# marc345/Dense2Sparse-ViT

Hardware: AMD Instinct MI355X
Metric: training images/s, DeiT-S 224 keep_ratio=0.5 (dense-to-sparse ViT train step, teacher fwd + student fwd/bwd + AdamW) (higher is better)
Workload: dtype f32; 1 GPU; DeiT-Small 224x224 patch16, 1-stage prune keep_ratio=0.5 @ block 3 (196->98 tokens), large LN predictor, kl_div mask loss, per-GPU batch 128; global_batch=128, parallelism=dp1

## Files before the change

dense2sparse-vit_amd/csrc/attention_f32.hip:

```cpp
#include "d2s_common.h"

namespace {

#ifdef D2S_ATTN_STAMPS
__device__ unsigned long long g_attn_stamps[16 * 8192];
#define ASTAMP(i) if (threadIdx.x == 0) { const int L_ = blockIdx.y * gridDim.x + blockIdx.x; if (L_ < 8192) g_attn_stamps[16 * L_ + (i)] = __builtin_amdgcn_s_memtime(); }
#define ASTAMPR(i) if (threadIdx.x == 0) { const int L_ = blockIdx.y * gridDim.x + blockIdx.x; if (L_ < 8192) g_attn_stamps[16 * L_ + (i)] = __builtin_amdgcn_s_memrealtime(); }
#else
#define ASTAMP(i)
#define ASTAMPR(i)
#endif

constexpr int DH = 64;
constexpr int PITCH = 68;

__device__ __forceinline__ void load_rows_regs(const float* __restrict__ base, long ld, int row, int nrows, int half,
                                               float scale, f32x4 (&r)[8]) {
    if (row < nrows) {
        const float* p = base + (long)row * ld + 4 * half;
#pragma unroll
        for (int t = 0; t < 8; ++t) {
            r[t] = *reinterpret_cast<const f32x4*>(p + 8 * t);
#pragma unroll
            for (int j = 0; j < 4; ++j) r[t][j] *= scale;
        }
    } else {
#pragma unroll
        for (int t = 0; t < 8; ++t) r[t] = f32x4{0.f, 0.f, 0.f, 0.f};
    }
}

__device__ __forceinline__ void tile_load(const float* __restrict__ base, long ld, int row0, int nrows, int tid, f32x4 (&r)[2]) {
#pragma unroll
    for (int i = 0; i < 2; ++i) {
        const int f = tid + i * 256, row = row0 + (f >> 4), d4 = (f & 15) * 4;
        r[i] = row < nrows ? *reinterpret_cast<const f32x4*>(base + (long)row * ld + d4) : f32x4{0.f, 0.f, 0.f, 0.f};
    }
}
__device__ __forceinline__ void tile_store(float* __restrict__ S, int tid, const f32x4 (&r)[2]) {
#pragma unroll
    for (int i = 0; i < 2; ++i) {
        const int f = tid + i * 256;
        *reinterpret_cast<f32x4*>(&S[(f >> 4) * PITCH + (f & 15) * 4]) = r[i];
    }
}

__device__ __forceinline__ void mma_lds_reg(const float* __restrict__ S, int l31, int half, const f32x4 (&y)[8], f32x16& acc) {
#pragma unroll
    for (int t = 0; t < 8; ++t) {
        const f32x4 a = *reinterpret_cast<const f32x4*>(&S[l31 * PITCH + 8 * t + 4 * half]);
#pragma unroll
        for (int j = 0; j < 4; ++j) acc = mfma32(a[j], y[t][j], acc);
    }
}
__device__ __forceinline__ void mma_reg_lds(const f32x16& p, const float* __restrict__ S, int l31, int half, f32x16 (&o)[2],
                                            int groups = 4) {
#pragma unroll
    for (int g = 0; g < 4; ++g) {
        if (g < groups) {
#pragma unroll
            for (int r = 4 * g; r < 4 * g + 4; ++r) {
                const float* row = &S[mfma32_row(r, half) * PITCH];
                o[0] = mfma32(p[r], row[l31], o[0]);
                o[1] = mfma32(p[r], row[32 + l31], o[1]);
            }
        }
    }
}

__device__ __forceinline__ void mma_lds_reg_t(const f32x16& p, const float* __restrict__ S, int l31, int half, f32x16 (&o)[2],
                                              int groups = 4) {
#pragma unroll
    for (int g = 0; g < 4; ++g) {
        if (g < groups) {
#pragma unroll
            for (int r = 4 * g; r < 4 * g + 4; ++r) {
                const float* row = &S[mfma32_row(r, half) * PITCH];
                o[0] = mfma32(row[l31], p[r], o[0]);
                o[1] = mfma32(row[32 + l31], p[r], o[1]);
            }
        }
    }
}

struct AttnFwdArgs {
    const float* qkv; float* out; float* lse; float* cls_row;
    const float* policy; float* cinv; const int* cu;
    int n, H; float scale, eps; int total;
};

template <bool POLICY, bool VARLEN>
__global__ __launch_bounds__(256, 3) void attn_fwd_kernel(AttnFwdArgs a) {
    __shared__ __attribute__((aligned(16))) float Ks[32 * PITCH];
    __shared__ __attribute__((aligned(16))) float Vs[32 * PITCH];
    __shared__ float pol_s[32];
    __shared__ __attribute__((aligned(16))) float vred[POLICY ? 16 * 64 : 4];
    __shared__ float vsum_s[64];
    extern __shared__ __attribute__((aligned(16))) float cls_s[];
    const int tid = threadIdx.x, lane = tid & 63, wave = tid >> 6, half = lane >> 5, l31 = lane & 31;
    const int H = a.H;
    ASTAMP(0); ASTAMPR(8);
    int bx, by;
    xcd_remap_2d(bx, by);
    const int b = by / H, h = by % H;
    const long ld = 3L * H * DH;
    const int row_base = VARLEN ? a.cu[b] : 0;
    const int n = VARLEN ? a.cu[b + 1] - row_base : a.n;
    if (VARLEN && bx * 128 >= n) return;
    const long tok0 = VARLEN ? (long)row_base : (long)b * n;
    const float* qb = a.qkv + tok0 * ld + h * DH;
    const float* kb = qb + (long)H * DH;
    const float* vb = kb + (long)H * DH;
    const float* polb = POLICY ? a.policy + (long)b * n : nullptr;
    const float scale = a.scale;
    const int q0 = bx * 128 + wave * 32;
    const bool active = q0 < n;
    const bool want_cls = a.cls_row != nullptr && bx == 0 && wave == 0;
    const int qi = q0 + l31;

    f32x4 qreg[8];
    load_rows_regs(qb, ld, qi, n, half, scale, qreg);

    f32x16 o[2];
#pragma unroll
    for (int r = 0; r < 16; ++r) { o[0][r] = 0.f; o[1][r] = 0.f; }
    float m_run = -INFINITY, l_run = 0.f;
    f32x4 vacc = {0.f, 0.f, 0.f, 0.f};

    const int ntiles = (n + 31) / 32;
    f32x4 kr[2], vr[2];
    float pr = 0.f;
    tile_load(kb, ld, 0, n, tid, kr);
    tile_load(vb, ld, 0, n, tid, vr);
    if (POLICY && tid < 32) pr = tid < n ? polb[tid] : 0.f;
    for (int t = 0; t < ntiles; ++t) {
        __syncthreads();
        tile_store(Ks, tid, kr);
        tile_store(Vs, tid, vr);
        if (POLICY) {
            if (tid < 32) pol_s[tid] = pr;
            vacc += vr[0];
            vacc += vr[1];
        }
        __syncthreads();
        if (t == 0) { ASTAMP(1); }
        if (t == 1) { ASTAMP(2); }
        if (t == 2) { ASTAMP(3); }
        if (t + 1 < ntiles) {
            tile_load(kb, ld, (t + 1) * 32, n, tid, kr);
            tile_load(vb, ld, (t + 1) * 32, n, tid, vr);
            if (POLICY && tid < 32) { const int kj = (t + 1) * 32 + tid; pr = kj < n ? polb[kj] : 0.f; }
        }
        if (!active) continue;
        f32x16 s;
#pragma unroll
        for (int r = 0; r < 16; ++r) s[r] = 0.f;
        mma_lds_reg(Ks, l31, half, qreg, s);
        const int kv0 = t * 32;
        float mt = -INFINITY;
#pragma unroll
        for (int r = 0; r < 16; ++r) {
            if (kv0 + mfma32_row(r, half) >= n) s[r] = -INFINITY;
            mt = fmaxf(mt, s[r]);
        }
        if (want_cls && l31 == 0) {
#pragma unroll
            for (int r = 0; r < 16; ++r) {
                const int key = kv0 + mfma32_row(r, half);
                if (key < n) cls_s[key] = s[r];
            }
        }
        mt = fmaxf(mt, __shfl_xor(mt, 32, 64));
        const float m_new = fmaxf(m_run, mt);
        const float alpha = __expf(m_run - m_new);
        float rs = 0.f;
#pragma unroll
        for (int r = 0; r < 16; ++r) {
            s[r] = __expf(s[r] - m_new);
            if (POLICY) {
                const int kr_ = mfma32_row(r, half);
                s[r] *= (kv0 + kr_ == qi) ? 1.f : pol_s[kr_];
            }
            rs += s[r];
        }
        rs += __shfl_xor(rs, 32, 64);
        l_run = l_run * alpha + rs;
        m_run = m_new;
#pragma unroll
        for (int r = 0; r < 16; ++r) {
            o[0][r] *= alpha;
            o[1][r] *= alpha;
        }
        mma_lds_reg_t(s, Vs, l31, half, o, min(4, (n - kv0 + 7) >> 3));
    }
    ASTAMP(4);
    const float c = POLICY ? a.eps / (float)n : 0.f;
    if (POLICY) {
        *reinterpret_cast<f32x4*>(&vred[(tid >> 4) * 64 + (tid & 15) * 4]) = vacc;
        __syncthreads();
        if (tid < 64) {
            float t = 0.f;
#pragma unroll
            for (int g = 0; g < 16; ++g) t += vred[g * 64 + tid];
            vsum_s[tid] = t * c;
        }
        __syncthreads();
    }
    if (!active) return;
    const float inv_l = 1.0f / (POLICY ? l_run + a.eps : l_run);
    if (qi < n) {
        float* p = a.out + (tok0 + qi) * H * DH + h * DH;
#pragma unroll
        for (int dt = 0; dt < 2; ++dt)
#pragma unroll
            for (int g = 0; g < 4; ++g) {
                f32x4 v;
#pragma unroll
                for (int j = 0; j < 4; ++j) {
                    float num = o[dt][4 * g + j];
                    if (POLICY) num += vsum_s[32 * dt + 8 * g + 4 * half + j];
                    v[j] = num * inv_l;
                }
                *reinterpret_cast<f32x4*>(p + 32 * dt + 8 * g + 4 * half) = v;
            }
    }
    const long stat0 = VARLEN ? (long)h * a.total + row_base : ((long)b * H + h) * n;
    if (half == 0 && qi < n) {
        if (a.lse) a.lse[stat0 + qi] = m_run + logf(POLICY ? l_run + a.eps : l_run);
        if (POLICY && a.cinv) a.cinv[stat0 + qi] = c * inv_l;
    }
    if (want_cls) {
        const float m0 = __shfl(m_run, 0, 64), il0 = __shfl(inv_l, 0, 64);
        float* cr = a.cls_row + stat0;
        for (int j = lane; j < n; j += 64) {
            float e = expf(cls_s[j] - m0);
            if (POLICY) e = e * (j == 0 ? 1.f : polb[j]) + c;
            cr[j] = e * il0;
        }
    }
    ASTAMP(5); ASTAMPR(9);
}

__global__ __launch_bounds__(256) void attn_delta_kernel(const float* __restrict__ out, const float* __restrict__ dout,
                                                         float* __restrict__ delta, long rows, int n, int H) {
    const int lane = threadIdx.x & 63;
    const long row = (long)blockIdx.x * 4 + (threadIdx.x >> 6);
    if (row >= rows) return;
    const long b = row / n, i = row - b * n;
    for (int h = 0; h < H; ++h) {
        const long e = row * H * DH + h * DH + lane;
        const float s = wave_sum(out[e] * dout[e]);
        if (lane == 0) delta[(b * H + h) * n + i] = s;
    }
}

template <bool POLICY>
__global__ __launch_bounds__(256, 3) void attn_bwd_dq_kernel(const float* __restrict__ qkv, const float* __restrict__ dout,
                                                          const float* __restrict__ lse, const float* __restrict__ delta,
                                                          float* __restrict__ dqkv, int n, int H, float scale,
                                                          const float* __restrict__ policy) {
    __shared__ __attribute__((aligned(16))) float Ks[32 * PITCH];
    __shared__ __attribute__((aligned(16))) float Vs[32 * PITCH];
    __shared__ float pol_s[32];
    const int tid = threadIdx.x, lane = tid & 63, wave = tid >> 6, half = lane >> 5, l31 = lane & 31;
    int bx, by;
    xcd_remap_2d(bx, by);
    const int b = by / H, h = by % H;
    const long ld = 3L * H * DH, ldo = (long)H * DH;
    const float* qb = qkv + (long)b * n * ld + h * DH;
    const float* kb = qb + (long)H * DH;
    const float* vb = kb + (long)H * DH;
    const float* dob = dout + (long)b * n * ldo + h * DH;
    const int q0 = bx * 128 + wave * 32;
    const bool active = q0 < n;

    f32x4 qreg[8], doreg[8];
    load_rows_regs(qb, ld, q0 + l31, n, half, scale, qreg);
    load_rows_regs(dob, ldo, q0 + l31, n, half, 1.0f, doreg);
    const bool qok = q0 + l31 < n;
    const float lse_i = qok ? lse[((long)b * H + h) * n + q0 + l31] : INFINITY;
    const float dl_i = qok ? delta[((long)b * H + h) * n + q0 + l31] : 0.f;

    f32x16 dq[2];
#pragma unroll
    for (int r = 0; r < 16; ++r) { dq[0][r] = 0.f; dq[1][r] = 0.f; }

    const int ntiles = (n + 31) / 32;
    f32x4 kr[2], vr[2];
    float pr = 0.f;
    const float* polb = POLICY ? policy + (long)b * n : nullptr;
    tile_load(kb, ld, 0, n, tid, kr);
    tile_load(vb, ld, 0, n, tid, vr);
    if (POLICY && tid < 32) pr = tid < n ? polb[tid] : 0.f;
    for (int t = 0; t < ntiles; ++t) {
        __syncthreads();
        tile_store(Ks, tid, kr);
        tile_store(Vs, tid, vr);
        if (POLICY && tid < 32) pol_s[tid] = pr;
        __syncthreads();
        if (t + 1 < ntiles) {
            tile_load(kb, ld, (t + 1) * 32, n, tid, kr);
            tile_load(vb, ld, (t + 1) * 32, n, tid, vr);
            if (POLICY && tid < 32) { const int kj = (t + 1) * 32 + tid; pr = kj < n ? polb[kj] : 0.f; }
        }
        if (!active) continue;
        f32x16 s, dp;
#pragma unroll
        for (int r = 0; r < 16; ++r) { s[r] = 0.f; dp[r] = 0.f; }
        mma_lds_reg(Ks, l31, half, qreg, s);
        mma_lds_reg(Vs, l31, half, doreg, dp);
        const int kv0 = t * 32;
#pragma unroll
        for (int r = 0; r < 16; ++r) {
            const int kr_ = mfma32_row(r, half);
            float p = (kv0 + kr_ < n) ? __expf(s[r] - lse_i) : 0.f;
            if (POLICY) p *= (kv0 + kr_ == q0 + l31) ? 1.f : pol_s[kr_];
            s[r] = p * (dp[r] - dl_i);
        }
        mma_reg_lds(s, Ks, l31, half, dq, min(4, (n - kv0 + 7) >> 3));
    }
    if (!active) return;
    float* dqb = dqkv + (long)b * n * ld + h * DH;
#pragma unroll
    for (int r = 0; r < 16; ++r) {
        const int qi = q0 + mfma32_row(r, half);
        if (qi < n) {
            float* p = dqb + (long)qi * ld;
            p[l31] = dq[0][r] * scale;
            p[32 + l31] = dq[1][r] * scale;
        }
    }
}

template <bool POLICY>
__global__ __launch_bounds__(256, 2) void attn_bwd_dkv_kernel(const float* __restrict__ qkv, const float* __restrict__ dout,
                                                           const float* __restrict__ lse, const float* __restrict__ delta,
                                                           float* __restrict__ dqkv, int n, int H, float scale,
                                                           const float* __restrict__ policy, const float* __restrict__ cinv) {
    __shared__ __attribute__((aligned(16))) float Qs[32 * PITCH];
    __shared__ __attribute__((aligned(16))) float Ds[32 * PITCH];
    __shared__ float lse_s[32], dl_s[32], ci_s[32];
    const int tid = threadIdx.x, lane = tid & 63, wave = tid >> 6, half = lane >> 5, l31 = lane & 31;
    int bx, by;
    xcd_remap_2d(bx, by);
    const int b = by / H, h = by % H;
    const long ld = 3L * H * DH, ldo = (long)H * DH;
    const float* qb = qkv + (long)b * n * ld + h * DH;
    const float* kb = qb + (long)H * DH;
    const float* vb = kb + (long)H * DH;
    const float* dob = dout + (long)b * n * ldo + h * DH;
    const float* lse_b = lse + ((long)b * H + h) * n;
    const float* dl_b = delta + ((long)b * H + h) * n;
    const int k0 = bx * 128 + wave * 32;
    const bool active = k0 < n;

    f32x4 kreg[8], vreg[8];
    load_rows_regs(kb, ld, k0 + l31, n, half, scale, kreg);
    load_rows_regs(vb, ld, k0 + l31, n, half, 1.0f, vreg);

    f32x16 dk[2], dv[2];
#pragma unroll
    for (int r = 0; r < 16; ++r) { dk[0][r] = 0.f; dk[1][r] = 0.f; dv[0][r] = 0.f; dv[1][r] = 0.f; }

    const int ntiles = (n + 31) / 32;
    f32x4 qr[2], dr[2];
    float lr = 0.f, dlr = 0.f, cir = 0.f;
    const float* ci_b = POLICY ? cinv + ((long)b * H + h) * n : nullptr;
    const float pol_key = (POLICY && k0 + l31 < n) ? policy[(long)b * n + k0 + l31] : 0.f;
    tile_load(qb, ld, 0, n, tid, qr);
    tile_load(dob, ldo, 0, n, tid, dr);
    if (tid < 32) { lr = tid < n ? lse_b[tid] : INFINITY; dlr = tid < n ? dl_b[tid] : 0.f; if (POLICY) cir = tid < n ? ci_b[tid] : 0.f; }
    for (int t = 0; t < ntiles; ++t) {
        __syncthreads();
        tile_store(Qs, tid, qr);
        tile_store(Ds, tid, dr);
        if (tid < 32) { lse_s[tid] = lr; dl_s[tid] = dlr; if (POLICY) ci_s[tid] = cir; }
        __syncthreads();
        if (t + 1 < ntiles) {
            tile_load(qb, ld, (t + 1) * 32, n, tid, qr);
            tile_load(dob, ldo, (t + 1) * 32, n, tid, dr);
            if (tid < 32) {
                const int qi = (t + 1) * 32 + tid;
                lr = qi < n ? lse_b[qi] : INFINITY;
                dlr = qi < n ? dl_b[qi] : 0.f;
                if (POLICY) cir = qi < n ? ci_b[qi] : 0.f;
            }
        }
        if (!active) continue;
        f32x16 s, dp;
#pragma unroll
        for (int r = 0; r < 16; ++r) { s[r] = 0.f; dp[r] = 0.f; }
        mma_lds_reg(Qs, l31, half, kreg, s);
        mma_lds_reg(Ds, l31, half, vreg, dp);
#pragma unroll
        for (int r = 0; r < 16; ++r) {
            const int qi = mfma32_row(r, half);
            float p = __expf(s[r] - lse_s[qi]);
            if (POLICY) p *= (t * 32 + qi == k0 + l31) ? 1.f : pol_key;
            s[r] = POLICY ? p + ci_s[qi] : p;
            dp[r] = p * (dp[r] - dl_s[qi]);
        }
        const int qgroups = min(4, (n - t * 32 + 7) >> 3);
        mma_reg_lds(s, Ds, l31, half, dv, qgroups);
        mma_reg_lds(dp, Qs, l31, half, dk, qgroups);
    }
    if (!active) return;
    float* dkb = dqkv + (long)b * n * ld + (long)H * DH + h * DH;
    float* dvb = dkb + (long)H * DH;
#pragma unroll
    for (int r = 0; r < 16; ++r) {
        const int ki = k0 + mfma32_row(r, half);
        if (ki < n) {
            float* pk = dkb + (long)ki * ld;
            float* pv = dvb + (long)ki * ld;
            pk[l31] = dk[0][r] * scale;
            pk[32 + l31] = dk[1][r] * scale;
            pv[l31] = dv[0][r];
            pv[32 + l31] = dv[1][r];
        }
    }
}

}

#ifdef D2S_ATTN_STAMPS
extern "C" int d2s_debug_read_attn_stamps(unsigned long long* host_out, int n_wg) {
    return hipMemcpyFromSymbol(host_out, HIP_SYMBOL(g_attn_stamps), (size_t)n_wg * 16 * sizeof(unsigned long long)) == hipSuccess ? 0 : -1;
}
#endif

extern "C" {

int d2s_attn_fwd_f32(const float* qkv, float* out, float* lse, float* cls_row, int B, int n, int H, float scale,
                     hipStream_t stream) {
    if (!qkv || !out || !lse || B <= 0 || n <= 0 || H <= 0 || n > 8192) return D2S_ERR_ARG;
    dim3 grid((n + 127) / 128, B * H), block(256);
    AttnFwdArgs a{qkv, out, lse, cls_row, nullptr, nullptr, nullptr, n, H, scale, 0.f, 0};
    hipLaunchKernelGGL((attn_fwd_kernel<false, false>), grid, block, cls_row ? (size_t)n * sizeof(float) : 0, stream, a);
    return d2s_check_launch();
}

int d2s_attn_policy_fwd_f32(const float* qkv, const float* policy, float* out, float* lse, float* cinv, float* cls_row, int B, int n,
                            int H, float scale, float eps, hipStream_t stream) {
    if (!qkv || !policy || !out || !lse || !cinv || B <= 0 || n <= 0 || H <= 0 || n > 8192) return D2S_ERR_ARG;
    dim3 grid((n + 127) / 128, B * H), block(256);
    AttnFwdArgs a{qkv, out, lse, cls_row, policy, cinv, nullptr, n, H, scale, eps, 0};
    hipLaunchKernelGGL((attn_fwd_kernel<true, false>), grid, block, cls_row ? (size_t)n * sizeof(float) : 0, stream, a);
    return d2s_check_launch();
}

int d2s_attn_varlen_fwd_f32(const float* qkv, const int* cu_seqlens, float* out, float* cls_row, int B, int total, int max_n, int H,
                            float scale, hipStream_t stream) {
    if (!qkv || !cu_seqlens || !out || B <= 0 || total <= 0 || max_n <= 0 || max_n > 8192 || H <= 0) return D2S_ERR_ARG;
    dim3 grid((max_n + 127) / 128, B * H), block(256);
    AttnFwdArgs a{qkv, out, nullptr, cls_row, nullptr, nullptr, cu_seqlens, 0, H, scale, 0.f, total};
    hipLaunchKernelGGL((attn_fwd_kernel<false, true>), grid, block, cls_row ? (size_t)max_n * sizeof(float) : 0, stream, a);
    return d2s_check_launch();
}

int d2s_attn_delta(const float* out, const float* dout, float* delta, int B, int n, int H, hipStream_t stream) {
    if (!out || !dout || !delta || B <= 0 || n <= 0 || H <= 0) return D2S_ERR_ARG;
    const long rows = (long)B * n;
    hipLaunchKernelGGL(attn_delta_kernel, dim3((unsigned)((rows + 3) / 4)), dim3(256), 0, stream, out, dout, delta, rows, n, H);
    return d2s_check_launch();
}

int d2s_attn_bwd_f32(const float* qkv, const float* out, const float* dout, const float* lse, float* dqkv, float* delta_ws, int B,
                     int n, int H, float scale, hipStream_t stream) {
    if (!qkv || !out || !dout || !lse || !dqkv || !delta_ws || B <= 0 || n <= 0 || H <= 0) return D2S_ERR_ARG;
    const long rows = (long)B * n;
    hipLaunchKernelGGL(attn_delta_kernel, dim3((unsigned)((rows + 3) / 4)), dim3(256), 0, stream, out, dout, delta_ws, rows, n, H);
    dim3 grid((n + 127) / 128, B * H), block(256);
    hipLaunchKernelGGL(attn_bwd_dq_kernel<false>, grid, block, 0, stream, qkv, dout, lse, delta_ws, dqkv, n, H, scale,
                       static_cast<const float*>(nullptr));
    hipLaunchKernelGGL(attn_bwd_dkv_kernel<false>, grid, block, 0, stream, qkv, dout, lse, delta_ws, dqkv, n, H, scale,
                       static_cast<const float*>(nullptr), static_cast<const float*>(nullptr));
    return d2s_check_launch();
}

int d2s_attn_policy_bwd_f32(const float* qkv, const float* policy, const float* out, const float* dout, const float* lse,
                            const float* cinv, float* dqkv, float* delta_ws, int B, int n, int H, float scale, hipStream_t stream) {
    if (!qkv || !policy || !out || !dout || !lse || !cinv || !dqkv || !delta_ws || B <= 0 || n <= 0 || H <= 0) return D2S_ERR_ARG;
    const long rows = (long)B * n;
    hipLaunchKernelGGL(attn_delta_kernel, dim3((unsigned)((rows + 3) / 4)), dim3(256), 0, stream, out, dout, delta_ws, rows, n, H);
    dim3 grid((n + 127) / 128, B * H), block(256);
    hipLaunchKernelGGL(attn_bwd_dq_kernel<true>, grid, block, 0, stream, qkv, dout, lse, delta_ws, dqkv, n, H, scale, policy);
    hipLaunchKernelGGL(attn_bwd_dkv_kernel<true>, grid, block, 0, stream, qkv, dout, lse, delta_ws, dqkv, n, H, scale, policy, cinv);
    return d2s_check_launch();
}

}
```

dense2sparse-vit_amd/csrc/d2s_common.h:

```cpp
#pragma once
#include <hip/hip_runtime.h>
#include <stdint.h>

#define D2S_OK 0
#define D2S_ERR_ARG (-1)
#define D2S_ERR_WORKSPACE (-2)
#define D2S_ERR_LAUNCH (-3)

#define D2S_WAVE 64

typedef float f32x4 __attribute__((ext_vector_type(4)));
typedef float f32x16 __attribute__((ext_vector_type(16)));

static inline int d2s_check_launch() { return hipGetLastError() == hipSuccess ? D2S_OK : D2S_ERR_LAUNCH; }

__device__ __forceinline__ float wave_sum(float v) {
#pragma unroll
    for (int o = 32; o > 0; o >>= 1) v += __shfl_xor(v, o, 64);
    return v;
}
__device__ __forceinline__ float wave_max(float v) {
#pragma unroll
    for (int o = 32; o > 0; o >>= 1) v = fmaxf(v, __shfl_xor(v, o, 64));
    return v;
}
__device__ __forceinline__ int wave_sum_i(int v) {
#pragma unroll
    for (int o = 32; o > 0; o >>= 1) v += __shfl_xor(v, o, 64);
    return v;
}
__device__ __forceinline__ float half_sum(float v) {
#pragma unroll
    for (int o = 16; o > 0; o >>= 1) v += __shfl_xor(v, o, 64);
    return v;
}

__device__ __forceinline__ f32x16 mfma32(float a, float b, f32x16 c) {
    return __builtin_amdgcn_mfma_f32_32x32x2f32(a, b, c, 0, 0, 0);
}
__device__ __forceinline__ int mfma32_row(int r, int half) { return (r & 3) + 8 * (r >> 2) + 4 * half; }

__device__ __forceinline__ float gelu_erf(float x) { return 0.5f * x * (1.0f + erff(x * 0.70710678118654752440f)); }
__device__ __forceinline__ float gelu_erf_grad(float x) {
    const float cdf = 0.5f * (1.0f + erff(x * 0.70710678118654752440f));
    const float pdf = 0.39894228040143267794f * __expf(-0.5f * x * x);
    return cdf + x * pdf;
}

__device__ __forceinline__ void xcd_remap_2d(int& bx, int& by) {
#ifdef D2S_NO_XCD_REMAP_2D
    bx = (int)blockIdx.x; by = (int)blockIdx.y;
    return;
#endif
    const int gx = (int)gridDim.x, total = gx * (int)gridDim.y;
    const int L = (int)blockIdx.y * gx + (int)blockIdx.x;
    const int xcd = L & 7, idx = L >> 3, q = total >> 3, r = total & 7;
    const int V = (xcd < r ? xcd * (q + 1) : r * (q + 1) + (xcd - r) * q) + idx;
    by = V / gx;
    bx = V - by * gx;
}

__device__ __forceinline__ void philox_round(uint32_t (&c)[4], uint32_t (&k)[2]) {
    const uint64_t p0 = (uint64_t)0xD2511F53u * c[0], p1 = (uint64_t)0xCD9E8D57u * c[2];
    const uint32_t n0 = (uint32_t)(p1 >> 32) ^ c[1] ^ k[0], n1 = (uint32_t)p1, n2 = (uint32_t)(p0 >> 32) ^ c[3] ^ k[1], n3 = (uint32_t)p0;
    c[0] = n0; c[1] = n1; c[2] = n2; c[3] = n3;
    k[0] += 0x9E3779B9u; k[1] += 0xBB67AE85u;
}
```

Before: 3591 images/s.

## Double-buffer attention LDS tiles and merge dq/dkv backward into one launch

Forward and both backward attention kernels now keep two LDS buffers for the K/V (or Q/dO) tiles, so each loop iteration needs one barrier instead of two and the next tile is stored while the current one is consumed. The separate dq and dkv backward kernels are merged into one launch whose blocks pick a role from a linear block index, with the XCD remap generalised to take a linear index. This removes one kernel launch and lets dq and dkv work share the GPU at the same time. In exchange it doubles LDS per block, which may lower occupancy, and the merged kernel runs the dq role under the dkv kernel's launch bounds of 2 blocks instead of 3.

```diff
diff --git a/dense2sparse-vit_amd/csrc/attention_f32.hip b/dense2sparse-vit_amd/csrc/attention_f32.hip
--- a/dense2sparse-vit_amd/csrc/attention_f32.hip
+++ b/dense2sparse-vit_amd/csrc/attention_f32.hip
@@ -13,6 +13,8 @@
 
 constexpr int DH = 64;
 constexpr int PITCH = 68;
+constexpr int TILE = 32 * PITCH;
+
 
 __device__ __forceinline__ void load_rows_regs(const float* __restrict__ base, long ld, int row, int nrows, int half,
                                                float scale, f32x4 (&r)[8]) {
@@ -91,9 +93,9 @@
 
 template <bool POLICY, bool VARLEN>
 __global__ __launch_bounds__(256, 3) void attn_fwd_kernel(AttnFwdArgs a) {
-    __shared__ __attribute__((aligned(16))) float Ks[32 * PITCH];
-    __shared__ __attribute__((aligned(16))) float Vs[32 * PITCH];
-    __shared__ float pol_s[32];
+    __shared__ __attribute__((aligned(16))) float Ks[2][TILE];
+    __shared__ __attribute__((aligned(16))) float Vs[2][TILE];
+    __shared__ float pol_s[2][32];
     __shared__ __attribute__((aligned(16))) float vred[POLICY ? 16 * 64 : 4];
     __shared__ float vsum_s[64];
     extern __shared__ __attribute__((aligned(16))) float cls_s[];
@@ -133,65 +135,71 @@
     tile_load(kb, ld, 0, n, tid, kr);
     tile_load(vb, ld, 0, n, tid, vr);
     if (POLICY && tid < 32) pr = tid < n ? polb[tid] : 0.f;
-    for (int t = 0; t < ntiles; ++t) {
-        __syncthreads();
-        tile_store(Ks, tid, kr);
-        tile_store(Vs, tid, vr);
+    auto stage = [&](int t1) {
+        tile_store(Ks[t1 & 1], tid, kr);
+        tile_store(Vs[t1 & 1], tid, vr);
         if (POLICY) {
-            if (tid < 32) pol_s[tid] = pr;
+            if (tid < 32) pol_s[t1 & 1][tid] = pr;
             vacc += vr[0];
             vacc += vr[1];
         }
+        if (t1 + 1 < ntiles) {
+            tile_load(kb, ld, (t1 + 1) * 32, n, tid, kr);
+            tile_load(vb, ld, (t1 + 1) * 32, n, tid, vr);
+            if (POLICY && tid < 32) { const int kj = (t1 + 1) * 32 + tid; pr = kj < n ? polb[kj] : 0.f; }
+        }
+    };
+    stage(0);
+    for (int t = 0; t < ntiles; ++t) {
         __syncthreads();
         if (t == 0) { ASTAMP(1); }
         if (t == 1) { ASTAMP(2); }
         if (t == 2) { ASTAMP(3); }
-        if (t + 1 < ntiles) {
-            tile_load(kb, ld, (t + 1) * 32, n, tid, kr);
-            tile_load(vb, ld, (t + 1) * 32, n, tid, vr);
-            if (POLICY && tid < 32) { const int kj = (t + 1) * 32 + tid; pr = kj < n ? polb[kj] : 0.f; }
-        }
-        if (!active) continue;
-        f32x16 s;
-#pragma unroll
-        for (int r = 0; r < 16; ++r) s[r] = 0.f;
-        mma_lds_reg(Ks, l31, half, qreg, s);
-        const int kv0 = t * 32;
-        float mt = -INFINITY;
-#pragma unroll
-        for (int r = 0; r < 16; ++r) {
-            if (kv0 + mfma32_row(r, half) >= n) s[r] = -INFINITY;
-            mt = fmaxf(mt, s[r]);
-        }
-        if (want_cls && l31 == 0) {
+        if (active) {
+            const float* Kc = Ks[t & 1];
+            const float* Vc = Vs[t & 1];
+            f32x16 s;
+#pragma unroll
+            for (int r = 0; r < 16; ++r) s[r] = 0.f;
+            mma_lds_reg(Kc, l31, half, qreg, s);
+            const int kv0 = t * 32;
+            float mt = -INFINITY;
 #pragma unroll
             for (int r = 0; r < 16; ++r) {
-                const int key = kv0 + mfma32_row(r, half);
-                if (key < n) cls_s[key] = s[r];
-            }
-        }
-        mt = fmaxf(mt, __shfl_xor(mt, 32, 64));
-        const float m_new = fmaxf(m_run, mt);
-        const float alpha = __expf(m_run - m_new);
-        float rs = 0.f;
-#pragma unroll
-        for (int r = 0; r < 16; ++r) {
-            s[r] = __expf(s[r] - m_new);
-            if (POLICY) {
-                const int kr_ = mfma32_row(r, half);
-                s[r] *= (kv0 + kr_ == qi) ? 1.f : pol_s[kr_];
-            }
-            rs += s[r];
-        }
-        rs += __shfl_xor(rs, 32, 64);
-        l_run = l_run * alpha + rs;
-        m_run = m_new;
-#pragma unroll
-        for (int r = 0; r < 16; ++r) {
-            o[0][r] *= alpha;
-            o[1][r] *= alpha;
-        }
-        mma_lds_reg_t(s, Vs, l31, half, o, min(4, (n - kv0 + 7) >> 3));
+                if (kv0 + mfma32_row(r, half) >= n) s[r] = -INFINITY;
+                mt = fmaxf(mt, s[r]);
+            }
+            if (want_cls && l31 == 0) {
+#pragma unroll
+                for (int r = 0; r < 16; ++r) {
+                    const int key = kv0 + mfma32_row(r, half);
+                    if (key < n) cls_s[key] = s[r];
+                }
+            }
+            mt = fmaxf(mt, __shfl_xor(mt, 32, 64));
+            const float m_new = fmaxf(m_run, mt);
+            const float alpha = __expf(m_run - m_new);
+            float rs = 0.f;
+#pragma unroll
+            for (int r = 0; r < 16; ++r) {
+                s[r] = __expf(s[r] - m_new);
+                if (POLICY) {
+                    const int kr_ = mfma32_row(r, half);
+                    s[r] *= (kv0 + kr_ == qi) ? 1.f : pol_s[t & 1][kr_];
+                }
+                rs += s[r];
+            }
+            rs += __shfl_xor(rs, 32, 64);
+            l_run = l_run * alpha + rs;
+            m_run = m_new;
+#pragma unroll
+            for (int r = 0; r < 16; ++r) {
+                o[0][r] *= alpha;
+                o[1][r] *= alpha;
+            }
+            mma_lds_reg_t(s, Vc, l31, half, o, min(4, (n - kv0 + 7) >> 3));
+        }
+        if (t + 1 < ntiles) stage(t + 1);
     }
     ASTAMP(4);
     const float c = POLICY ? a.eps / (float)n : 0.f;
@@ -254,17 +262,23 @@
     }
 }
 
+struct AttnBwdArgs {
+    const float* qkv; const float* dout; const float* lse; const float* delta; float* dqkv;
+    const float* policy; const float* cinv;
+    int n, H; float scale;
+};
+constexpr int BWD_ROWV = 3 * 32;
+constexpr int BWD_SMEM = 2 * (2 * TILE + BWD_ROWV);
+
 template <bool POLICY>
-__global__ __launch_bounds__(256, 3) void attn_bwd_dq_kernel(const float* __restrict__ qkv, const float* __restrict__ dout,
-                                                          const float* __restrict__ lse, const float* __restrict__ delta,
-                                                          float* __restrict__ dqkv, int n, int H, float scale,
-                                                          const float* __restrict__ policy) {
-    __shared__ __attribute__((aligned(16))) float Ks[32 * PITCH];
-    __shared__ __attribute__((aligned(16))) float Vs[32 * PITCH];
-    __shared__ float pol_s[32];
+__device__ __forceinline__ void attn_bwd_dq_role(const AttnBwdArgs& a, float* __restrict__ smem, int bx, int by) {
+    float* Ks = smem;
+    float* Vs = smem + 2 * TILE;
+    float* pol_s = smem + 4 * TILE;
+    const float* __restrict__ qkv = a.qkv; const float* __restrict__ dout = a.dout; const float* __restrict__ lse = a.lse;
+    const float* __restrict__ delta = a.delta; float* __restrict__ dqkv = a.dqkv; const float* __restrict__ policy = a.policy;
+    const int n = a.n, H = a.H; const float scale = a.scale;
     const int tid = threadIdx.x, lane = tid & 63, wave = tid >> 6, half = lane >> 5, l31 = lane & 31;
-    int bx, by;
-    xcd_remap_2d(bx, by);
     const int b = by / H, h = by % H;
     const long ld = 3L * H * DH, ldo = (long)H * DH;
     const float* qb = qkv + (long)b * n * ld + h * DH;
@@ -292,32 +306,38 @@
     tile_load(kb, ld, 0, n, tid, kr);
     tile_load(vb, ld, 0, n, tid, vr);
     if (POLICY && tid < 32) pr = tid < n ? polb[tid] : 0.f;
+    auto stage = [&](int t1) {
+        tile_store(Ks + (t1 & 1) * TILE, tid, kr);
+        tile_store(Vs + (t1 & 1) * TILE, tid, vr);
+        if (POLICY && tid < 32) pol_s[(t1 & 1) * 32 + tid] = pr;
+        if (t1 + 1 < ntiles) {
+            tile_load(kb, ld, (t1 + 1) * 32, n, tid, kr);
+            tile_load(vb, ld, (t1 + 1) * 32, n, tid, vr);
+            if (POLICY && tid < 32) { const int kj = (t1 + 1) * 32 + tid; pr = kj < n ? polb[kj] : 0.f; }
+        }
+    };
+    stage(0);
     for (int t = 0; t < ntiles; ++t) {
         __syncthreads();
-        tile_store(Ks, tid, kr);
-        tile_store(Vs, tid, vr);
-        if (POLICY && tid < 32) pol_s[tid] = pr;
-        __syncthreads();
-        if (t + 1 < ntiles) {
-            tile_load(kb, ld, (t + 1) * 32, n, tid, kr);
-            tile_load(vb, ld, (t + 1) * 32, n, tid, vr);
-            if (POLICY && tid < 32) { const int kj = (t + 1) * 32 + tid; pr = kj < n ? polb[kj] : 0.f; }
-        }
-        if (!active) continue;
-        f32x16 s, dp;
-#pragma unroll
-        for (int r = 0; r < 16; ++r) { s[r] = 0.f; dp[r] = 0.f; }
-        mma_lds_reg(Ks, l31, half, qreg, s);
-        mma_lds_reg(Vs, l31, half, doreg, dp);
-        const int kv0 = t * 32;
-#pragma unroll
-        for (int r = 0; r < 16; ++r) {
-            const int kr_ = mfma32_row(r, half);
-            float p = (kv0 + kr_ < n) ? __expf(s[r] - lse_i) : 0.f;
-            if (POLICY) p *= (kv0 + kr_ == q0 + l31) ? 1.f : pol_s[kr_];
-            s[r] = p * (dp[r] - dl_i);
-        }
-        mma_reg_lds(s, Ks, l31, half, dq, min(4, (n - kv0 + 7) >> 3));
+        if (active) {
+            const float* Kc = Ks + (t & 1) * TILE;
+            const float* Vc = Vs + (t & 1) * TILE;
+            f32x16 s, dp;
+#pragma unroll
+            for (int r = 0; r < 16; ++r) { s[r] = 0.f; dp[r] = 0.f; }
+            mma_lds_reg(Kc, l31, half, qreg, s);
+            mma_lds_reg(Vc, l31, half, doreg, dp);
+            const int kv0 = t * 32;
+#pragma unroll
+            for (int r = 0; r < 16; ++r) {
+                const int kr_ = mfma32_row(r, half);
+                float p = (kv0 + kr_ < n) ? __expf(s[r] - lse_i) : 0.f;
+                if (POLICY) p *= (kv0 + kr_ == q0 + l31) ? 1.f : pol_s[(t & 1) * 32 + kr_];
+                s[r] = p * (dp[r] - dl_i);
+            }
+            mma_reg_lds(s, Kc, l31, half, dq, min(4, (n - kv0 + 7) >> 3));
+        }
+        if (t + 1 < ntiles) stage(t + 1);
     }
     if (!active) return;
     float* dqb = dqkv + (long)b * n * ld + h * DH;
@@ -333,16 +353,15 @@
 }
 
 template <bool POLICY>
-__global__ __launch_bounds__(256, 2) void attn_bwd_dkv_kernel(const float* __restrict__ qkv, const float* __restrict__ dout,
-                                                           const float* __restrict__ lse, const float* __restrict__ delta,
-                                                           float* __restrict__ dqkv, int n, int H, float scale,
-                                                           const float* __restrict__ policy, const float* __restrict__ cinv) {
-    __shared__ __attribute__((aligned(16))) float Qs[32 * PITCH];
-    __shared__ __attribute__((aligned(16))) float Ds[32 * PITCH];
-    __shared__ float lse_s[32], dl_s[32], ci_s[32];
+__device__ __forceinline__ void attn_bwd_dkv_role(const AttnBwdArgs& a, float* __restrict__ smem, int bx, int by) {
+    float* Qs = smem;
+    float* Ds = smem + 2 * TILE;
+    float* rowv = smem + 4 * TILE;
+    const float* __restrict__ qkv = a.qkv; const float* __restrict__ dout = a.dout; const float* __restrict__ lse = a.lse;
+    const float* __restrict__ delta = a.delta; float* __restrict__ dqkv = a.dqkv; const float* __restrict__ policy = a.policy;
+    const float* __restrict__ cinv = a.cinv;
+    const int n = a.n, H = a.H; const float scale = a.scale;
     const int tid = threadIdx.x, lane = tid & 63, wave = tid >> 6, half = lane >> 5, l31 = lane & 31;
-    int bx, by;
-    xcd_remap_2d(bx, by);
     const int b = by / H, h = by % H;
     const long ld = 3L * H * DH, ldo = (long)H * DH;
     const float* qb = qkv + (long)b * n * ld + h * DH;
@@ -370,39 +389,51 @@
     tile_load(qb, ld, 0, n, tid, qr);
     tile_load(dob, ldo, 0, n, tid, dr);
     if (tid < 32) { lr = tid < n ? lse_b[tid] : INFINITY; dlr = tid < n ? dl_b[tid] : 0.f; if (POLICY) cir = tid < n ? ci_b[tid] : 0.f; }
-    for (int t = 0; t < ntiles; ++t) {
-        __syncthreads();
-        tile_store(Qs, tid, qr);
-        tile_store(Ds, tid, dr);
-        if (tid < 32) { lse_s[tid] = lr; dl_s[tid] = dlr; if (POLICY) ci_s[tid] = cir; }
-        __syncthreads();
-        if (t + 1 < ntiles) {
-            tile_load(qb, ld, (t + 1) * 32, n, tid, qr);
-            tile_load(dob, ldo, (t + 1) * 32, n, tid, dr);
+    auto stage = [&](int t1) {
+        tile_store(Qs + (t1 & 1) * TILE, tid, qr);
+        tile_store(Ds + (t1 & 1) * TILE, tid, dr);
+        if (tid < 32) {
+            float* rv = rowv + (t1 & 1) * BWD_ROWV;
+            rv[tid] = lr; rv[32 + tid] = dlr; if (POLICY) rv[64 + tid] = cir;
+        }
+        if (t1 + 1 < ntiles) {
+            tile_load(qb, ld, (t1 + 1) * 32, n, tid, qr);
+            tile_load(dob, ldo, (t1 + 1) * 32, n, tid, dr);
             if (tid < 32) {
-                const int qi = (t + 1) * 32 + tid;
+                const int qi = (t1 + 1) * 32 + tid;
                 lr = qi < n ? lse_b[qi] : INFINITY;
                 dlr = qi < n ? dl_b[qi] : 0.f;
                 if (POLICY) cir = qi < n ? ci_b[qi] : 0.f;
             }
         }
-        if (!active) continue;
-        f32x16 s, dp;
-#pragma unroll
-        for (int r = 0; r < 16; ++r) { s[r] = 0.f; dp[r] = 0.f; }
-        mma_lds_reg(Qs, l31, half, kreg, s);
-        mma_lds_reg(Ds, l31, half, vreg, dp);
-#pragma unroll
-        for (int r = 0; r < 16; ++r) {
-            const int qi = mfma32_row(r, half);
-            float p = __expf(s[r] - lse_s[qi]);
-            if (POLICY) p *= (t * 32 + qi == k0 + l31) ? 1.f : pol_key;
-            s[r] = POLICY ? p + ci_s[qi] : p;
-            dp[r] = p * (dp[r] - dl_s[qi]);
-        }
-        const int qgroups = min(4, (n - t * 32 + 7) >> 3);
-        mma_reg_lds(s, Ds, l31, half, dv, qgroups);
-        mma_reg_lds(dp, Qs, l31, half, dk, qgroups);
+    };
+    stage(0);
+    for (int t = 0; t < ntiles; ++t) {
+        __syncthreads();
+        if (active) {
+            const float* Qc = Qs + (t & 1) * TILE;
+            const float* Dc = Ds + (t & 1) * TILE;
+            const float* lse_s = rowv + (t & 1) * BWD_ROWV;
+            const float* dl_s = lse_s + 32;
+            const float* ci_s = lse_s + 64;
+            f32x16 s, dp;
+#pragma unroll
+            for (int r = 0; r < 16; ++r) { s[r] = 0.f; dp[r] = 0.f; }
+            mma_lds_reg(Qc, l31, half, kreg, s);
+            mma_lds_reg(Dc, l31, half, vreg, dp);
+#pragma unroll
+            for (int r = 0; r < 16; ++r) {
+                const int qi = mfma32_row(r, half);
+                float p = __expf(s[r] - lse_s[qi]);
+                if (POLICY) p *= (t * 32 + qi == k0 + l31) ? 1.f : pol_key;
+                s[r] = POLICY ? p + ci_s[qi] : p;
+                dp[r] = p * (dp[r] - dl_s[qi]);
+            }
+            const int qgroups = min(4, (n - t * 32 + 7) >> 3);
+            mma_reg_lds(s, Dc, l31, half, dv, qgroups);
+            mma_reg_lds(dp, Qc, l31, half, dk, qgroups);
+        }
+        if (t + 1 < ntiles) stage(t + 1);
     }
     if (!active) return;
     float* dkb = dqkv + (long)b * n * ld + (long)H * DH + h * DH;
@@ -421,6 +452,28 @@
     }
 }
 
+template <bool POLICY>
+__global__ __launch_bounds__(256, 2) void attn_bwd_kernel(AttnBwdArgs a, int gx, int G) {
+    __shared__ __attribute__((aligned(16))) float smem[BWD_SMEM];
+    const int G8 = (G + 7) & ~7;
+    int L = (int)blockIdx.x;
+    const bool dkv_role = L < G8;
+    if (dkv_role && L >= G) return;
+    if (!dkv_role) L -= G8;
+    int bx, by;
+    xcd_remap_linear(L, gx, G, bx, by);
+    if (dkv_role) attn_bwd_dkv_role<POLICY>(a, smem, bx, by);
+    else attn_bwd_dq_role<POLICY>(a, smem, bx, by);
+}
+
+template <bool POLICY>
+int attn_bwd_launch(const AttnBwdArgs& a, int B, hipStream_t stream) {
+    const int gx = (a.n + 127) / 128, G = gx * B * a.H;
+    if ((long)gx * B * a.H > (1L << 30)) return D2S_ERR_ARG;
+    hipLaunchKernelGGL(attn_bwd_kernel<POLICY>, dim3(((G + 7) & ~7) + G), dim3(256), 0, stream, a, gx, G);
+    return d2s_check_launch();
+}
+
 }
 
 #ifdef D2S_ATTN_STAMPS
@@ -470,12 +523,7 @@
     if (!qkv || !out || !dout || !lse || !dqkv || !delta_ws || B <= 0 || n <= 0 || H <= 0) return D2S_ERR_ARG;
     const long rows = (long)B * n;
     hipLaunchKernelGGL(attn_delta_kernel, dim3((unsigned)((rows + 3) / 4)), dim3(256), 0, stream, out, dout, delta_ws, rows, n, H);
-    dim3 grid((n + 127) / 128, B * H), block(256);
-    hipLaunchKernelGGL(attn_bwd_dq_kernel<false>, grid, block, 0, stream, qkv, dout, lse, delta_ws, dqkv, n, H, scale,
-                       static_cast<const float*>(nullptr));
-    hipLaunchKernelGGL(attn_bwd_dkv_kernel<false>, grid, block, 0, stream, qkv, dout, lse, delta_ws, dqkv, n, H, scale,
-                       static_cast<const float*>(nullptr), static_cast<const float*>(nullptr));
-    return d2s_check_launch();
+    return attn_bwd_launch<false>(AttnBwdArgs{qkv, dout, lse, delta_ws, dqkv, nullptr, nullptr, n, H, scale}, B, stream);
 }
 
 int d2s_attn_policy_bwd_f32(const float* qkv, const float* policy, const float* out, const float* dout, const float* lse,
@@ -483,10 +531,7 @@
     if (!qkv || !policy || !out || !dout || !lse || !cinv || !dqkv || !delta_ws || B <= 0 || n <= 0 || H <= 0) return D2S_ERR_ARG;
     const long rows = (long)B * n;
     hipLaunchKernelGGL(attn_delta_kernel, dim3((unsigned)((rows + 3) / 4)), dim3(256), 0, stream, out, dout, delta_ws, rows, n, H);
-    dim3 grid((n + 127) / 128, B * H), block(256);
-    hipLaunchKernelGGL(attn_bwd_dq_kernel<true>, grid, block, 0, stream, qkv, dout, lse, delta_ws, dqkv, n, H, scale, policy);
-    hipLaunchKernelGGL(attn_bwd_dkv_kernel<true>, grid, block, 0, stream, qkv, dout, lse, delta_ws, dqkv, n, H, scale, policy, cinv);
-    return d2s_check_launch();
-}
-
-}
+    return attn_bwd_launch<true>(AttnBwdArgs{qkv, dout, lse, delta_ws, dqkv, policy, cinv, n, H, scale}, B, stream);
+}
+
+}
diff --git a/dense2sparse-vit_amd/csrc/d2s_common.h b/dense2sparse-vit_amd/csrc/d2s_common.h
--- a/dense2sparse-vit_amd/csrc/d2s_common.h
+++ b/dense2sparse-vit_amd/csrc/d2s_common.h
@@ -47,17 +47,19 @@
     return cdf + x * pdf;
 }
 
-__device__ __forceinline__ void xcd_remap_2d(int& bx, int& by) {
+__device__ __forceinline__ void xcd_remap_linear(int L, int gx, int total, int& bx, int& by) {
 #ifdef D2S_NO_XCD_REMAP_2D
-    bx = (int)blockIdx.x; by = (int)blockIdx.y;
+    by = L / gx; bx = L - by * gx;
     return;
 #endif
-    const int gx = (int)gridDim.x, total = gx * (int)gridDim.y;
-    const int L = (int)blockIdx.y * gx + (int)blockIdx.x;
     const int xcd = L & 7, idx = L >> 3, q = total >> 3, r = total & 7;
     const int V = (xcd < r ? xcd * (q + 1) : r * (q + 1) + (xcd - r) * q) + idx;
     by = V / gx;
     bx = V - by * gx;
+}
+__device__ __forceinline__ void xcd_remap_2d(int& bx, int& by) {
+    const int gx = (int)gridDim.x;
+    xcd_remap_linear((int)blockIdx.y * gx + (int)blockIdx.x, gx, gx * (int)gridDim.y, bx, by);
 }
 
 __device__ __forceinline__ void philox_round(uint32_t (&c)[4], uint32_t (&k)[2]) {
```

Result: no change. 3606 images/s, median of 6 (+0.4%).
